# asd56585452/IGS

Measured on AMD Instinct MI355X. Metric: Gaussians rendered/sec (fwd+bwd) at 1352x1014; PSNR vs ref, higher is better.
Workload: dtype f32

## Files before the change

igs_amd/_cabi.py:

```python
import ctypes as C
import os

from . import build as _build

_LIB = None
E_RETRY = -6

ALLOC_FN = C.CFUNCTYPE(C.c_void_p, C.c_void_p, C.c_size_t)
_vp, _i, _f = C.c_void_p, C.c_int, C.c_float

class RefineStepArgs(C.Structure):
    _fields_ = [("stream", C.c_void_p),
                ("geometry_buffer", ALLOC_FN), ("geometry_user", C.c_void_p),
                ("binning_buffer", ALLOC_FN), ("binning_user", C.c_void_p),
                ("image_buffer", ALLOC_FN), ("image_user", C.c_void_p),
                ("workspace", C.c_void_p),
                ("P", C.c_int), ("D", C.c_int), ("M", C.c_int), ("width", C.c_int), ("height", C.c_int),
                ("background", C.c_void_p),
                ("param", C.c_void_p), ("exp_avg", C.c_void_p), ("exp_avg_sq", C.c_void_p), ("grad_out", C.c_void_p),
                ("off_xyz", C.c_size_t), ("off_rot", C.c_size_t), ("off_sh", C.c_size_t), ("off_opacity", C.c_size_t),
                ("off_scale", C.c_size_t),
                ("lr_xyz", C.c_float), ("lr_rot", C.c_float), ("lr_sh", C.c_float), ("lr_opacity", C.c_float), ("lr_scale", C.c_float),
                ("beta1", C.c_float), ("beta2", C.c_float), ("eps", C.c_float),
                ("step", C.c_int),
# ... 20 lines not shown

SIGNATURES = {
    "igs_rast_version": (_i, []),
    "igs_rast_last_error": (C.c_char_p, []),
    "igs_rast_forward": (_i, _FORWARD),
    "igs_rast_forward_async": (_i, _FORWARD),
    "igs_rast_forward_finish": (_i, []),
    "igs_rast_forward_nowait": (_i, _FORWARD),
    "igs_rast_last_status": (_i, _STATUS),
    "igs_rast_last_posted_status": (_i, _STATUS),
    "igs_rast_hint_scratch_clean": (None, [_i]),
    "igs_rast_count_gaussians": (_i, ([_vp, ALLOC_FN, _vp, ALLOC_FN, _vp, ALLOC_FN, _vp, _i, _i, _i, _vp, _i, _i]
                                      + [_vp] * 5 + [_f, _vp, _vp, _vp, _vp, _vp, _f, _f, _i] + [_vp] * 4 + [_i])),
    "igs_rast_set_slab_hint": (None, [_u]),
    "igs_rast_get_slab_hint": (_u, []),
    "igs_rast_backward_workspace_bytes": (_sz, [_i]),
    "igs_rast_backward": (_i, ([_vp, _i, _i, _i, _i, _vp, _i, _i] + [_vp] * 5 + [_f, _vp, _vp, _vp, _vp, _vp, _f, _f, _f]
                               + [_vp] * 5 + [_vp] * 7 + [_vp] + [_vp] * 8 + [_i, _i, _i])),
    "igs_rast_mark_visible": (_i, [_vp, _i, _vp, _vp, _vp, _vp]),
    "igs_rast_debug_dump": (_i, [_vp, _i, _i, _i, _i] + [_vp] * 8),
    "igs_rast_next_backward_options": (None, [_i, _f]),
    "igs_rast_nan_report_wait": (_i, []),
    "igs_rast_nan_report_handle": (_i, [_vp, _vp]),
    "igs_rast_nan_report_wait_at": (_i, [_vp, _u]),
    "igs_rast_last_backward_instance": (_i, []),
    "igs_rast_debug_poison_lds": (_i, [_vp]),
    "igs_rast_profile_enable": (_i, [_i]),
    "igs_rast_profile_read": (_i, [_vp, _vp, _vp, _vp, _i]),
    "igs_adam_step": (_i, [_vp, _sz, _vp, _vp, _vp, _vp, _f, _f, _f, _f, _f, _f]),
    "igs_adam_step_groups": (_i, [_vp, _i, _vp, _vp, _vp, _vp, _vp, _vp, _vp, _f, _f, _f, _f, _f]),
# ... 137 lines not shown
```

igs_amd/csrc/api.hip:

```cpp
#include <atomic>
#include "common.h"
#include "host_api.h"
#include <math.h>
#include <stdio.h>
#include <string.h>
#include <stdlib.h>
#include <time.h>

static thread_local char g_err[512] = "";
int fail(int code, const char* what, hipError_t e)
{
    if (e != hipSuccess) snprintf(g_err, sizeof g_err, "%s: %s", what, hipGetErrorString(e));
    else snprintf(g_err, sizeof g_err, "%s", what);
    return code;
}
int fail_in(const char* fn, const char* what)
{
    snprintf(g_err, sizeof g_err, "%s: %s", fn, what);
    return IGS_RAST_E_INVALID;
}
static const bool g_trace_launches = getenv("IGS_TRACE_LAUNCHES") != nullptr;
#define DBG_SYNC(what) do { if (debug || g_trace_launches) { hipError_t e_ = hipStreamSynchronize(s); if (e_ != hipSuccess) return fail(IGS_RAST_E_HIP, what, e_); \
                                                              if (g_trace_launches) { fprintf(stderr, "[igs] completed: %s\n", what); fflush(stderr); } } } while (0)

// ... 101 lines not shown
    if (r_sum) *r_sum = g_prof.r_sum;
    if (calls) *calls = g_prof.calls;
    if (reset) { for (int i = 0; i < ST_COUNT; i++) { g_prof.ms[i] = 0; g_prof.cnt[i] = 0; } g_prof.r_sum = 0; g_prof.calls = 0; }
    return ST_COUNT;
}

extern "C" int igs_rast_version(void) { return IGS_RAST_VERSION; }
extern "C" const char* igs_rast_last_error(void) { return g_err; }
static inline size_t ws_gacc_bytes(int P) { return ((size_t)(P > 0 ? P : 0) * GACC_F * 8 + 255) & ~(size_t)255; }
#define WS_LOSS_BYTES 4096
extern "C" size_t igs_rast_backward_workspace_bytes(int P) { return ws_gacc_bytes(P) + WS_LOSS_BYTES + 512; }

struct BinHint { uint32_t slab = 0; };
#define SLAB_MAX_BYTES (8ull << 30)
static thread_local BinHint g_hint;
static uint32_t slab_hint_for(uint32_t overflow)
{
    const uint64_t want = ((uint64_t)overflow + overflow / 4 + 255) / 256 * 256;
    return (uint32_t)(want > TILE_SORT_BIG ? TILE_SORT_BIG : want);
}
struct PendingFwd { bool active = false; uint32_t slab = 0; };
static thread_local PendingFwd g_pending;

struct FwdIn {
    hipStream_t s; igs_rast_alloc_fn geometry_buffer; void* geometry_user; igs_rast_alloc_fn binning_buffer; void* binning_user;
    igs_rast_alloc_fn image_buffer; void* image_user; int P, D, M; const float* background; int width, height;
    const float *means3D, *shs, *colors_precomp, *opacities, *scales; float scale_modifier; const float *rotations, *cov3D_precomp;
    const float *viewmatrix, *projmatrix, *cam_pos; float tan_fovx, tan_fovy, kernel_size; int prefiltered;
    float *out_color, *out_coord, *out_mcoord, *out_depth, *out_mdepth, *out_alpha, *out_normal; int* radii; int require_coord, require_depth, debug;
};
// ... 196 lines not shown
    if (b.pending) { g_host_seq = g_host_seq + 1 ? g_host_seq + 1 : 1; g_slot.pinned[3] = 0; }
    ba.host_seq = g_host_seq;
    if (b.pending && ex.no_latch) g_nowait_seq = g_host_seq;
    g_status_stream = s;
    if (ex.fused_ran) *ex.fused_ran = b.fuse_tiles;
    if (ex.count) {
        ba.tile_order = nullptr;
        HIP_TRY(launch_blend_count(s, ba, ex.count), "blend_count launch");
    } else if (b.fuse_tiles) {
        BlendBwdArgs& bb = *ex.fused_bwd;
        bb.W = in.width; bb.H = in.height; bb.gx = f.gx; bb.gy = f.gy; bb.fx = f.fp.fx; bb.fy = f.fp.fy; bb.bg = in.background;
        bb.ranges = b.ranges; bb.point_list = b.point_list; bb.rec = f.rec(); bb.colors_precomp = nullptr;
        bb.tile_order = nullptr;
        ba.tile_order = nullptr;
        if (b.step_order) { ba.step_order = f.ibuf(f.IL.tile_order); ba.reset_cursors = f.ibuf(f.IL.tile_count); }
        HIP_TRY(launch_blend_step(s, ba, bb, in.require_coord != 0, in.require_depth != 0, ex.fused_instance), "blend_step launch");
        if (b.step_order) g_counters_dirty = false;
    } else {
        HIP_TRY(launch_blend_fwd(s, ba, in.require_coord != 0, in.require_depth != 0), "blend_fwd launch");
    }
    DBG_SYNC("blend_fwd");
    prof_mark(s, ST_BLEND_FWD);
    return 0;
}

struct FrameStatus { uint32_t R, overflow, prefilter; };
static FrameStatus read_status(const uint32_t* p) { return { __atomic_load_n(&p[0], __ATOMIC_ACQUIRE), __atomic_load_n(&p[1], __ATOMIC_ACQUIRE), p[2] }; }
static int collect_status(hipStream_t s, uint32_t* overflow)
{
    if (int rc = wait_status(s)) return rc;
    const FrameStatus st = read_status(g_slot.pinned);
// ... 130 lines not shown
    const uint32_t seq = __atomic_load_n(&p[3], __ATOMIC_ACQUIRE);
    if (check_seq && seq != (g_nowait_seq ? g_nowait_seq : g_host_seq))
        return fail(IGS_RAST_E_RETRY, "igs_rast_last_status: the captured forward has not posted its status yet (replay the graph and synchronise the stream first)");
    const FrameStatus st = read_status(p);
    if (num_rendered) *num_rendered = st.R > 0x7FFFFFFFu ? 0x7FFFFFFF : (int)st.R;
    if (overflow) *overflow = st.overflow;
    if (prefilter_flag) *prefilter_flag = st.prefilter;
    if (st.overflow && slab_hint_for(st.overflow) > g_hint.slab) g_hint.slab = slab_hint_for(st.overflow);
    return 0;
}
extern "C" int igs_rast_last_status(int* num_rendered, unsigned* overflow, unsigned* prefilter) { return last_status(num_rendered, overflow, prefilter, true); }
extern "C" int igs_rast_last_posted_status(int* num_rendered, unsigned* overflow, unsigned* prefilter) { return last_status(num_rendered, overflow, prefilter, false); }

extern "C" void igs_rast_set_slab_hint(unsigned slots_per_tile) { g_hint.slab = slots_per_tile > TILE_SORT_BIG ? TILE_SORT_BIG : slots_per_tile; }
extern "C" unsigned igs_rast_get_slab_hint(void) { return g_hint.slab; }

static int g_last_bwd_instance = -1;
extern "C" int igs_rast_last_backward_instance(void) { return __atomic_load_n(&g_last_bwd_instance, __ATOMIC_RELAXED); }

#define NAN_RING 256
struct NanTicket { volatile uint32_t* word = nullptr; hipEvent_t ev = nullptr; uint32_t seq = 0; };
struct NanSlot { uint32_t* pinned = nullptr; uint32_t* pinned_dev = nullptr; NanTicket* tickets = nullptr; uint32_t seq = 0; bool requested = false; bool pending = false; };
static thread_local NanSlot g_nan[IGS_MAX_DEVICES];
static thread_local int g_nan_dev = -1;
static thread_local float g_next_clamp = 0.f;
extern "C" void igs_rast_next_backward_options(int nan_report, float clamp_grads)
{
    g_next_clamp = clamp_grads > 0.f ? clamp_grads : 0.f;
    int dev = 0;
    if (hipGetDevice(&dev) != hipSuccess || dev < 0 || dev >= IGS_MAX_DEVICES) return;
// ... 415 lines not shown
```

igs_amd/csrc/blend_bwd.hip:

```cpp
#include "blend_bwd_tile.h"

template <bool COORD, bool DEPTH, bool NORMAL, bool ABS = true, bool MASK = false>
__global__ void __launch_bounds__(256)
blend_bwd_kernel(const BlendBwdArgs a)
{
    using Cfg = BwdCfg<COORD, DEPTH, NORMAL, ABS>;
    __shared__ float4 chunk[Cfg::BCHUNK * Cfg::NQ];
    __shared__ uint32_t chunk_id[Cfg::BCHUNK];
    __shared__ uint64_t quad_bits[4][Cfg::NSW];
    __shared__ int wave_max[4];
    __shared__ __attribute__((aligned(16))) float red[Cfg::RED_FLOATS];

    uint32_t tile;
    if (a.tile_order && a.tile_order[a.gx * a.gy] == 1u) {
        if (blockIdx.x >= (uint32_t)(a.gx * a.gy)) return;
        tile = a.tile_order[blockIdx.x];
        if (tile >= (uint32_t)(a.gx * a.gy)) return;
    } else if (!tile_for_block(blockIdx.x, a.gx, a.gy, tile)) return;
    blend_bwd_tile<COORD, DEPTH, NORMAL, ABS, false, MASK>(a, tile, chunk, chunk_id, quad_bits, wave_max, red, nullptr);
}

hipError_t launch_blend_bwd(hipStream_t s, const BlendBwdArgs& a, bool coord, bool depth, bool* compact_layout, int* instance_bits)
{
    const dim3 grid(tile_grid_blocks(a.gx, a.gy)), block(256);
    const bool C = coord && (a.dL_dcoord || a.dL_dmcoord);
    const bool D = depth && (a.dL_ddepth || a.dL_dmdepth);
    const bool N = (coord || depth) && a.dL_dnormal;
    if (compact_layout) *compact_layout = !C && !D && !N;
    if (instance_bits) *instance_bits = (C ? 1 : 0) | (D ? 2 : 0) | (N ? 4 : 0) | ((C || (D && !N) || (!D && N) || a.want_absgrad) ? 8 : 0);
    if (a.first_trainable > 0) {
        if (C || a.want_absgrad || (D != N)) return hipErrorInvalidValue;
        if (D) hipLaunchKernelGGL((blend_bwd_kernel<false, true, true, false, true>), grid, block, 0, s, a);
        else   hipLaunchKernelGGL((blend_bwd_kernel<false, false, false, false, true>), grid, block, 0, s, a);
        return hipGetLastError();
// ... 14 lines not shown
```

igs_amd/csrc/blend_bwd_tile.h:

```cpp
#pragma once
#include "blend_common.h"
#include "blend_fwd_tile.h"

#define BCHUNK_MAX 128

template <int STRIDE_B, int R0, int N> struct ColWrite;
template <int STRIDE_B, int R0> struct ColWrite<STRIDE_B, R0, 1> {
    static __device__ __forceinline__ void run(unsigned m0, const float* v) {
        asm volatile("s_mov_b32 m0, %1\n\ts_nop 0\n\tds_write_addtid_b32 %0 offset:%2" :: "v"(v[R0]), "s"(m0), "n"(R0 * STRIDE_B) : "memory", "m0");
    }
};
template <int STRIDE_B, int R0> struct ColWrite<STRIDE_B, R0, 2> {
    static __device__ __forceinline__ void run(unsigned m0, const float* v) {
        asm volatile("s_mov_b32 m0, %2\n\ts_nop 0\n\tds_write_addtid_b32 %0 offset:%3\n\tds_write_addtid_b32 %1 offset:%4"
                     :: "v"(v[R0]), "v"(v[R0 + 1]), "s"(m0), "n"(R0 * STRIDE_B), "n"((R0 + 1) * STRIDE_B) : "memory", "m0");
    }
};
template <int STRIDE_B, int R0> struct ColWrite<STRIDE_B, R0, 3> {
    static __device__ __forceinline__ void run(unsigned m0, const float* v) {
        asm volatile("s_mov_b32 m0, %3\n\ts_nop 0\n\tds_write_addtid_b32 %0 offset:%4\n\tds_write_addtid_b32 %1 offset:%5\n\tds_write_addtid_b32 %2 offset:%6"
                     :: "v"(v[R0]), "v"(v[R0 + 1]), "v"(v[R0 + 2]), "s"(m0), "n"(R0 * STRIDE_B), "n"((R0 + 1) * STRIDE_B), "n"((R0 + 2) * STRIDE_B) : "memory", "m0");
    }
};
template <int STRIDE_B, int R0> struct ColWrite<STRIDE_B, R0, 4> {
// ... 34 lines not shown
        ColWrite<STRIDE_B, R0, 5>::run(m0, v);
        ColWrite<STRIDE_B, R0 + 5, N - 5>::run(m0, v);
    }
};

#define BWD_RED_STRIDE 68
template <bool COORD, bool DEPTH, bool NORMAL, bool ABS> struct BwdCfg {
    static constexpr bool GEO = COORD || DEPTH || NORMAL;
    static constexpr int NQ = GEO ? 6 : 3;
    static constexpr int BCHUNK = GEO ? 64 : 128;
    static constexpr int NSW = BCHUNK / 64;
    static constexpr int NROWS = 9 + (ABS ? 1 : 0) + (COORD ? 9 : 0) + (DEPTH ? 3 : 0) + (NORMAL ? 3 : 0);
    static constexpr int RED_FLOATS = 4 * NROWS * BWD_RED_STRIDE;
};

template <bool COORD, bool DEPTH, bool NORMAL, bool ABS, bool PRE, bool MASK = false>
__device__ __forceinline__ void blend_bwd_tile(const BlendBwdArgs& a, const uint32_t tile, float4* __restrict__ chunk, uint32_t* __restrict__ chunk_id,
                                               uint64_t (*quad_bits)[BwdCfg<COORD, DEPTH, NORMAL, ABS>::NSW], int* wave_max,
                                               float* __restrict__ red_all, const FwdPix* pre)
{
    constexpr bool GEO = COORD || DEPTH || NORMAL;
    constexpr int NQ = BwdCfg<COORD, DEPTH, NORMAL, ABS>::NQ;
    constexpr int BCHUNK = BwdCfg<COORD, DEPTH, NORMAL, ABS>::BCHUNK;
    constexpr int NSW = BwdCfg<COORD, DEPTH, NORMAL, ABS>::NSW;
    constexpr int NROWS = BwdCfg<COORD, DEPTH, NORMAL, ABS>::NROWS;
    constexpr int RED_STRIDE = BWD_RED_STRIDE;
    constexpr uint32_t SEG_ROT = NROWS == 9 ? 0x1b46bu
                               : NROWS == 10 ? 0x4431eu
                               : NROWS == 16 ? 0xa7dbb9c7u
                               : 0u;
    const uint32_t tx = tile % a.gx, ty = tile / a.gx;
    const uint32_t tid = threadIdx.x, lane = tid & 63, wid = tid >> 6;
    const uint32_t px = tx * TILE + (wid & 1) * 8 + (lane & 7);
    const uint32_t py = ty * TILE + (wid >> 1) * 8 + (lane >> 3);
    const bool inside = px < (uint32_t)a.W && py < (uint32_t)a.H;
    const float pixfx = (float)px, pixfy = (float)py;
    const float tile_x0 = (float)(tx * TILE), tile_y0 = (float)(ty * TILE);
    const size_t HW = (size_t)a.H * a.W;
    const size_t pix = (size_t)a.W * py + px;

    const uint2 range = ((const uint2*)a.ranges)[tile];
    int last_contributor;
    if constexpr (PRE) last_contributor = inside ? (int)min(pre->last_contributor, range.y - range.x) : 0;
    else last_contributor = inside ? (int)min(a.n_contrib[pix], range.y - range.x) : 0;
    uint32_t max_contributor = 0u;
    if constexpr (COORD || DEPTH) max_contributor = inside ? a.n_contrib[pix + HW] : 0u;

    float gp0 = 0, gp1 = 0, gp2 = 0, g_alpha = 0, T_final = 0, bg_dot = 0;
    if (a.l1_gt) {
        float acc = 0.f;
        if (inside) {
            float c0, c1, c2;
            if constexpr (PRE) {
                c0 = pre->C0 + pre->T * a.bg[0]; c1 = pre->C1 + pre->T * a.bg[1]; c2 = pre->C2 + pre->T * a.bg[2];
            } else { c0 = a.l1_color[pix]; c1 = a.l1_color[HW + pix]; c2 = a.l1_color[2 * HW + pix]; }
            const float d0 = c0 - a.l1_gt[pix], d1 = c1 - a.l1_gt[HW + pix];
// ... 44 lines not shown
                    gn0 = (d0 - dt * n0) / nlen; gn1 = (d1 - dt * n1) / nlen; gn2 = (d2 - dt * n2) / nlen;
                }
            }
        }
    }

    int my_wave_max;
    {
        int m = last_contributor;
#pragma unroll
        for (int off = 32; off > 0; off >>= 1) m = max(m, __shfl_xor(m, off, 64));
        if (lane == 0) wave_max[wid] = m;
        my_wave_max = __builtin_amdgcn_readfirstlane(m);
    }
    tile_barrier();
    const int n = max(max(wave_max[0], wave_max[1]), max(wave_max[2], wave_max[3]));
    const int rounds = (n + BCHUNK - 1) / BCHUNK;

    float T = T_final, S = 0.f, Dprev = 0.f, last_alpha = 0.f;
    const bool has_bg = (a.bg[0] != 0.f) || (a.bg[1] != 0.f) || (a.bg[2] != 0.f);
    const float halfW = 0.5f * a.W, halfH = 0.5f * a.H;
    float* myred = red_all + wid * (NROWS * RED_STRIDE);
    const unsigned myred_m0 = (unsigned)__builtin_amdgcn_readfirstlane((int)(unsigned)(size_t)myred);
    constexpr int LPR = NROWS <= 16 ? 4 : 2;
#ifndef BWD_ADJ
#define BWD_ADJ 1
#endif
    constexpr bool ADJ = BWD_ADJ && LPR == 4 && NROWS < 16;
    const int rrow = ADJ ? (int)(lane >> 2) : (int)(lane & (64 / LPR - 1)), rpart = ADJ ? (int)(lane & 3) : (int)(lane / (64 / LPR));
    const int rseg = ADJ ? rpart : LPR == 4 ? ((rpart + (int)((SEG_ROT >> (2 * (rrow & 15))) & 3u)) & 3) : rpart;
// ... 172 lines not shown
```

igs_amd/csrc/blend_fwd.hip:

```cpp
#include "blend_fwd_tile.h"

template <bool COORD, bool DEPTH, bool NORMAL, bool LEAN = false>
__global__ void __launch_bounds__(256) __attribute__((amdgpu_waves_per_eu(8, 8)))
blend_fwd_kernel(const BlendFwdArgs a)
{
    constexpr bool GEO = COORD || DEPTH || NORMAL;
    __shared__ float4 chunk[FWD_CHUNK * (GEO ? 6 : 3)];
    __shared__ uint64_t quad_bits[FWD_NLIST][FWD_NSW];
    __shared__ int wave_done[4];
    __shared__ uint32_t order_hist[2 * LOAD_CLASSES];

    if (blockIdx.x == 0 && threadIdx.x == 0 && a.host_dst) {
        __hip_atomic_store(&a.host_dst[0], a.stats_src[0], __ATOMIC_RELAXED, __HIP_MEMORY_SCOPE_SYSTEM);
        __hip_atomic_store(&a.host_dst[1], a.stats_src[1], __ATOMIC_RELAXED, __HIP_MEMORY_SCOPE_SYSTEM);
        __hip_atomic_store(&a.host_dst[2], a.flag_src[0], __ATOMIC_RELAXED, __HIP_MEMORY_SCOPE_SYSTEM);
        asm volatile("s_waitcnt vmcnt(0)" ::: "memory");
        __hip_atomic_store(&a.host_dst[3], a.host_seq, __ATOMIC_RELAXED, __HIP_MEMORY_SCOPE_SYSTEM);
    }
    if (blockIdx.x == 0 && a.tile_order) build_tile_order(a.ranges, (uint32_t)(a.gx * a.gy), a.tile_order, order_hist);
    uint32_t tile;
    if (!tile_for_block(blockIdx.x, a.gx, a.gy, tile)) return;
    FwdPix px;
    blend_fwd_tile<COORD, DEPTH, NORMAL, LEAN, true>(a, tile, chunk, quad_bits, wave_done, px);
}

hipError_t launch_blend_fwd(hipStream_t s, const BlendFwdArgs& a, bool coord, bool depth)
{
    const dim3 grid(tile_grid_blocks(a.gx, a.gy)), block(256);
    if (a.skip_bwd_state && coord && depth) hipLaunchKernelGGL((blend_fwd_kernel<true, true, true, true>), grid, block, 0, s, a);
    else if (coord && depth) hipLaunchKernelGGL((blend_fwd_kernel<true, true, true>), grid, block, 0, s, a);
    else if (coord) hipLaunchKernelGGL((blend_fwd_kernel<true, false, true>), grid, block, 0, s, a);
    else if (depth) hipLaunchKernelGGL((blend_fwd_kernel<false, true, true>), grid, block, 0, s, a);
    else hipLaunchKernelGGL((blend_fwd_kernel<false, false, false>), grid, block, 0, s, a);
    return hipGetLastError();
}
```

igs_amd/csrc/blend_fwd_tile.h:

```cpp
#pragma once
#include "blend_common.h"

#define FWD_CHUNK 192
#define FWD_NSW (FWD_CHUNK / 64)
#define FWD_NLIST 4

struct FwdPix {
    float C0, C1, C2;
    float T;
    float weight;
    uint32_t last_contributor;
};

template <bool COORD, bool DEPTH, bool NORMAL, bool LEAN, bool KEEP_N>
__device__ __forceinline__ void blend_fwd_tile(const BlendFwdArgs& a, const uint32_t tile, float4* __restrict__ chunk,
                                               uint64_t (*quad_bits)[FWD_NSW], int* wave_done, FwdPix& px_out)
{
    constexpr bool GEO = COORD || DEPTH || NORMAL;
    constexpr int NQ = GEO ? 6 : 3;
    const uint32_t tx = tile % a.gx, ty = tile / a.gx;
    const uint32_t tid = threadIdx.x, lane = tid & 63, wid = tid >> 6;
    const uint32_t px = tx * TILE + (wid & 1) * 8 + (lane & 7);
    const uint32_t py = ty * TILE + (wid >> 1) * 8 + (lane >> 3);
    const bool inside = px < (uint32_t)a.W && py < (uint32_t)a.H;
    const float pixfx = (float)px, pixfy = (float)py;
    const float tile_x0 = (float)(tx * TILE), tile_y0 = (float)(ty * TILE);

    const uint2 range = ((const uint2*)a.ranges)[tile];
    const int n = (int)(range.y - range.x);
    const int rounds = (n + FWD_CHUNK - 1) / FWD_CHUNK;

    float T = 1.0f;
    float Tl = inside ? 1.0f : 0.0f;
    uint32_t last_contributor = 0, max_contributor = 0xFFFFFFFFu;
    float C0 = 0, C1 = 0, C2 = 0, weight = 0;
    float Co0 = 0, Co1 = 0, Co2 = 0, mC0 = 0, mC1 = 0, mC2 = 0, Depth = 0, mDepth = 0, N0 = 0, N1 = 0, N2 = 0;

    if (tid < 4) wave_done[tid] = 0;
    for (int i = 0; i < rounds; i++) {
        tile_barrier();
        if (wave_done[0] & wave_done[1] & wave_done[2] & wave_done[3]) break;
        const int progress = i * FWD_CHUNK + (int)tid;
        uint32_t qmask = 0;
        if (tid < FWD_CHUNK && progress < n) {
            const uint32_t id = a.point_list[range.x + progress];
            const float4* src = (const float4*)(a.rec + (size_t)id * REC_F);
            float4 q0 = src[0], q1 = src[1], q2 = src[2];
            if (a.colors_precomp) {
                q1.z = a.colors_precomp[3 * (size_t)id]; q1.w = a.colors_precomp[3 * (size_t)id + 1];
                q2.x = a.colors_precomp[3 * (size_t)id + 2];
            }
            chunk[tid * NQ + 0] = q0; chunk[tid * NQ + 1] = q1; chunk[tid * NQ + 2] = q2;
// ... 3 lines not shown
        if (wid < FWD_NSW) {
#pragma unroll
            for (int q = 0; q < FWD_NLIST; q++) {
                const uint64_t b = __ballot((qmask >> q) & 1u);
                if (lane == 0) quad_bits[q][wid] = b;
            }
        }
        tile_barrier();
        auto blend_row = [&](const float4* r, const auto slot) {
                    const float4 q0 = r[0], q1 = r[1], q2 = r[2];
                    const float dx = q0.x - pixfx, dy = q0.y - pixfy;
                    const float power = gauss_power(q0.z, q0.w, q1.x, dx, dy);
                    const float alpha = fminf(0.99f, q1.y * __expf(power));
                    const float alpha_e = (!(power > 0.0f) && !(alpha < 1.0f / 255.0f)) ? alpha : 0.0f;
                    const float test_T = Tl * (1.0f - alpha_e);
                    const bool alive = !(test_T < 0.0001f);
                    const float aT = alive ? alpha_e * Tl : 0.0f;
                    const bool contrib = aT > 0.0f;
                    const uint32_t contributor = (uint32_t)(i * FWD_CHUNK + 1) + (uint32_t)slot;
                    C0 += q1.z * aT; C1 += q1.w * aT; C2 += q2.x * aT;
                    if constexpr (GEO) {
                        const float4 q3 = r[3];
                        const float4 q5 = r[5];
                        if constexpr (COORD) {
                            const float4 q4 = r[4];
                            const float c0 = q3.x + q4.x * dx + q4.y * dy;
                            const float c1 = q3.y + q4.z * dx + q4.w * dy;
                            const float c2 = q3.z + q5.x * dx + q5.y * dy;
                            Co0 += c0 * aT; Co1 += c1 * aT; Co2 += c2 * aT;
                        }
                        if constexpr (DEPTH) {
// ... 6 lines not shown
                    weight += aT;
                    T = alive ? test_T : T;
                    Tl = alive ? test_T : 0.0f;
                    last_contributor = contrib ? contributor : last_contributor;
        };
        if (__ballot(Tl != 0.0f) != 0ull) {
            bool wave_finished = false;
            for (int sw = 0; sw < FWD_NSW && !wave_finished; sw++) {
                uint64_t bits = uniform64(quad_bits[wid][sw]);
                while (bits != 0ull) {
                    const int jj = __builtin_ctzll(bits);
                    asm("s_bitset0_b64 %0, %1" : "+s"(bits) : "s"(jj));
                    const int j = sw * 64 + jj;
                    uint32_t addr;
                    if constexpr (NQ * 16 <= 64) asm("v_mul_u32_u24 %0, %1, %2" : "=v"(addr) : "s"(j), "n"(NQ * 16));
                    else asm("v_mul_u32_u24 %0, %1, %2" : "=v"(addr) : "s"(j), "v"(NQ * 16));
                    blend_row((const float4*)((const char*)chunk + addr), (uint32_t)j);
                }
                if (__ballot(Tl != 0.0f) == 0ull) wave_finished = true;
            }
        }
        const bool all_done = __ballot(Tl != 0.0f) == 0ull;
        if (lane == 0) wave_done[wid] = all_done ? 1 : 0;
    }

    if (inside) {
        const size_t HW = (size_t)a.H * a.W;
        const size_t pix = (size_t)a.W * py + px;
        if constexpr (GEO) {
            if (max_contributor != 0xFFFFFFFFu) {
                const uint32_t id = a.point_list[range.x + max_contributor - 1];
// ... 60 lines not shown
```

igs_amd/csrc/blend_step.hip:

```cpp
#include "blend_fwd_tile.h"
#include "blend_bwd_tile.h"

#ifdef BLEND_TIMELINE
#define BLEND_TL_MARKS 4
#define BLEND_TL_WGS 16384
__device__ unsigned long long g_blend_tl[BLEND_TL_WGS * BLEND_TL_MARKS];
extern "C" int igs_debug_blend_timeline(unsigned long long* host, int n)
{
    return (int)hipMemcpyFromSymbol(host, HIP_SYMBOL(g_blend_tl), (size_t)n * 8);
}
#define BTL(k, val) do { if (threadIdx.x == 0 && blockIdx.x < BLEND_TL_WGS) g_blend_tl[blockIdx.x * BLEND_TL_MARKS + (k)] = (val); } while (0)
#else
#define BTL(k, val) do { } while (0)
#endif
template <bool COORD, bool DEPTH, bool NORMAL, bool ABS, bool MASK = false>
__global__ void __launch_bounds__(256) __attribute__((amdgpu_waves_per_eu(8, 8)))
blend_step_kernel(const BlendFwdArgs f, const BlendBwdArgs b)
{
    constexpr bool GEO = COORD || DEPTH || NORMAL;
    using Cfg = BwdCfg<false, false, false, ABS>;
    constexpr size_t FWD_BYTES = (size_t)FWD_CHUNK * (GEO ? 6 : 3) * 16;
    constexpr size_t BWD_CHUNK_BYTES = (size_t)Cfg::BCHUNK * Cfg::NQ * 16;
    constexpr size_t BWD_BYTES = BWD_CHUNK_BYTES + (size_t)Cfg::RED_FLOATS * 4;
    __shared__ __attribute__((aligned(16))) char smem[FWD_BYTES > BWD_BYTES ? FWD_BYTES : BWD_BYTES];
    __shared__ uint64_t quad_bits_f[FWD_NLIST][FWD_NSW];
    __shared__ uint64_t quad_bits_b[4][Cfg::NSW];
    __shared__ int wave_done[4];
    __shared__ int wave_max[4];

    if (blockIdx.x == 0 && threadIdx.x == 0 && f.host_dst) {
        __hip_atomic_store(&f.host_dst[0], f.stats_src[0], __ATOMIC_RELAXED, __HIP_MEMORY_SCOPE_SYSTEM);
        __hip_atomic_store(&f.host_dst[1], f.stats_src[1], __ATOMIC_RELAXED, __HIP_MEMORY_SCOPE_SYSTEM);
        __hip_atomic_store(&f.host_dst[2], f.flag_src[0], __ATOMIC_RELAXED, __HIP_MEMORY_SCOPE_SYSTEM);
        asm volatile("s_waitcnt vmcnt(0)" ::: "memory");
        __hip_atomic_store(&f.host_dst[3], f.host_seq, __ATOMIC_RELAXED, __HIP_MEMORY_SCOPE_SYSTEM);
    }
    uint32_t tile;
    BTL(0, wall_clock64());
    if (f.step_order) {
        tile = f.step_order[blockIdx.x];
        if (tile >= (uint32_t)(f.gx * f.gy)) return;
    } else if (!tile_for_block(blockIdx.x, f.gx, f.gy, tile)) return;
    if (f.reset_cursors && threadIdx.x == 0) f.reset_cursors[tile] = 0u;
    BTL(3, (unsigned long long)(f.ranges[2 * tile + 1] - f.ranges[2 * tile]));
    FwdPix px;
    blend_fwd_tile<COORD, DEPTH, NORMAL, true, false>(f, tile, (float4*)smem, quad_bits_f, wave_done, px);
    tile_barrier();
    BTL(1, wall_clock64());
    blend_bwd_tile<false, false, false, ABS, true, MASK>(b, tile, (float4*)smem, nullptr, quad_bits_b, wave_max, (float*)(smem + BWD_CHUNK_BYTES), &px);
    BTL(2, wall_clock64());
}

hipError_t launch_blend_step(hipStream_t s, const BlendFwdArgs& f, const BlendBwdArgs& b, bool coord, bool depth, int* instance_bits)
{
    if (!f.skip_bwd_state || !b.l1_gt || b.dL_dcoord || b.dL_dmcoord || b.dL_ddepth || b.dL_dmdepth || b.dL_dnormal || b.dL_dalpha || b.colors_precomp)
        return hipErrorInvalidValue;
    const dim3 grid(tile_grid_blocks(f.gx, f.gy)), block(256);
    if (instance_bits) *instance_bits = b.want_absgrad ? 8 : 0;
    if (b.first_trainable > 0) {
        if (b.want_absgrad) return hipErrorInvalidValue;
        if (coord && depth) hipLaunchKernelGGL((blend_step_kernel<true, true, true, false, true>), grid, block, 0, s, f, b);
        else if (!coord && !depth) hipLaunchKernelGGL((blend_step_kernel<false, false, false, false, true>), grid, block, 0, s, f, b);
        else return hipErrorInvalidValue;
        return hipGetLastError();
    }
    if (coord && depth) {
        if (b.want_absgrad) hipLaunchKernelGGL((blend_step_kernel<true, true, true, true>), grid, block, 0, s, f, b);
        else hipLaunchKernelGGL((blend_step_kernel<true, true, true, false>), grid, block, 0, s, f, b);
    } else if (!coord && !depth) {
        if (b.want_absgrad) hipLaunchKernelGGL((blend_step_kernel<false, false, false, true>), grid, block, 0, s, f, b);
        else hipLaunchKernelGGL((blend_step_kernel<false, false, false, false>), grid, block, 0, s, f, b);
    } else return hipErrorInvalidValue;
    return hipGetLastError();
}
```

igs_amd/csrc/common.h:

```cpp
#pragma once
#include <hip/hip_runtime.h>
#include <stdint.h>
#include <stddef.h>

#define TILE 16
#define TILE_PIX 256
#define CHUNK 256

#define REC_F 32
#define REC_BLEND_F 24

#define GACC_F 32
#define GACC_COMPACT_F 16
enum { GA_COLOR = 0, GA_VP = 3, GA_CP = 6, GA_TS = 12, GA_RP = 13, GA_NRM = 15, GA_M2D = 18, GA_M2DZ = 20,
       GA_CONIC = 21, GA_OPA = 24, GA_USED = 25 };

static inline size_t align_up(size_t x, size_t a) { return (x + a - 1) / a * a; }

#define COUNTER_SHARDS 64
#define COUNTER_SHARD_STRIDE 16
#define SORT_ITEMS 8
#define SORT_TILE (256 * SORT_ITEMS)
#define SORT_MAX_PASSES 5
#define SORT_MAX_BLOCKS 256
// ... 109 lines not shown
hipError_t launch_count_score(hipStream_t s, int P, const int* count, const float* opacities, float* score);

struct BlendBwdArgs {
    int W, H, gx, gy;
    float fx, fy; const float* bg;
    const uint32_t* ranges; const uint32_t* point_list; const float* rec; const float* colors_precomp;
    const float *alphas, *normalmap, *accum_coord, *accum_depth, *normal_length; const uint32_t* n_contrib;
    const float *dL_dpix, *dL_dcoord, *dL_dmcoord, *dL_ddepth, *dL_dmdepth, *dL_dalpha, *dL_dnormal;
    double* gacc;
    const float *l1_color, *l1_gt; float l1_scale; float* l1_loss;
    int want_absgrad = 1;
    const uint32_t* tile_order = nullptr;
    int first_trainable = 0;
};
hipError_t launch_blend_bwd(hipStream_t s, const BlendBwdArgs& a, bool coord, bool depth, bool* compact_layout, int* instance_bits = nullptr);
hipError_t launch_blend_step(hipStream_t s, const BlendFwdArgs& f, const BlendBwdArgs& b, bool coord, bool depth, int* instance_bits = nullptr);

struct GeomBwdArgs {
    int P, D, M, W, H;
    const float *means3D, *shs, *scales, *rotations, *cov3D_precomp; const int* radii;
    float scale_modifier, tan_fovx, tan_fovy, fx, fy, kernel_size;
    const float *view, *proj, *campos;
    const float* rec; const double* gacc;
    int gacc_compact;
    float *dL_dmean2D, *dL_dcolor, *dL_dopacity, *dL_dmean3D, *dL_dcov3D, *dL_dsh, *dL_dscale, *dL_drot;
    uint32_t* nan_host = nullptr; uint32_t nan_seq = 0;
    float clamp = 0.f;
    const float* plane_cache = nullptr; uint32_t plane_tag = 0;
};
hipError_t launch_geom_bwd(hipStream_t s, const GeomBwdArgs& a);

// ... 183 lines not shown
```

include/igs_rast.h:

```cpp
#ifndef IGS_RAST_H
#define IGS_RAST_H

#include <stddef.h>
#include <stdint.h>

#ifdef __cplusplus
extern "C" {
#endif

#define IGS_RAST_VERSION 4

#define IGS_RAST_E_INVALID   (-1)
#define IGS_RAST_E_HIP       (-2)
#define IGS_RAST_E_ALLOC     (-3)
#define IGS_RAST_E_PREFILTER (-4)
#define IGS_RAST_E_CHANNELS  (-5)

#define IGS_RAST_E_RETRY     (-6)

typedef char* (*igs_rast_alloc_fn)(void* user, size_t bytes);

int igs_rast_version(void);
const char* igs_rast_last_error(void);

// ... 76 lines not shown
    const float* rotations,
    const float* cov3D_precomp,
    const float* viewmatrix,
    const float* projmatrix,
    const float* cam_pos,
    float tan_fovx, float tan_fovy,
    int prefiltered,
    float* out_color,
    int* count,
    float* score,
    int* radii,
    int debug);

void igs_rast_set_slab_hint(unsigned slots_per_tile);
unsigned igs_rast_get_slab_hint(void);

size_t igs_rast_backward_workspace_bytes(int P);

int igs_rast_backward(
    void* stream,
    int P, int D, int M, int R,
    const float* background,
    int width, int height,
    const float* means3D,
    const float* shs,
    const float* colors_precomp,
    const float* alphas,
    const float* scales,
    float scale_modifier,
    const float* rotations,
// ... 244 lines not shown
```

Before: 863.9 million.

## Turn fused blend step kernel into persistent tile loop with atomic ticket queues

The fused forward+backward blend kernel becomes persistent. The grid is sized to resident occupancy (CUs × blocks per CU), and workgroups pull tiles from eight sharded atomic ticket counters instead of launching one workgroup per tile. The next tile's range is prefetched with scalar loads after the backward barrier, and kernel arguments are reread from the kernarg segment through scalar loads to reduce register pressure. This aims to cut workgroup launch overhead and tail imbalance, but adds atomic contention and counter-reset logic that could fail at edge cases.

```diff
diff --git a/igs_amd/_cabi.py b/igs_amd/_cabi.py
--- a/igs_amd/_cabi.py
+++ b/igs_amd/_cabi.py
@@ -58,6 +58,7 @@
                                       + [_vp] * 5 + [_f, _vp, _vp, _vp, _vp, _vp, _f, _f, _i] + [_vp] * 4 + [_i])),
     "igs_rast_set_slab_hint": (None, [_u]),
     "igs_rast_get_slab_hint": (_u, []),
+    "igs_rast_set_step_grid": (_i, [_i]),
     "igs_rast_backward_workspace_bytes": (_sz, [_i]),
     "igs_rast_backward": (_i, ([_vp, _i, _i, _i, _i, _vp, _i, _i] + [_vp] * 5 + [_f, _vp, _vp, _vp, _vp, _vp, _f, _f, _f]
                                + [_vp] * 5 + [_vp] * 7 + [_vp] + [_vp] * 8 + [_i, _i, _i])),
diff --git a/igs_amd/csrc/api.hip b/igs_amd/csrc/api.hip
--- a/igs_amd/csrc/api.hip
+++ b/igs_amd/csrc/api.hip
@@ -139,6 +139,7 @@
 struct BinHint { uint32_t slab = 0; };
 #define SLAB_MAX_BYTES (8ull << 30)
 static thread_local BinHint g_hint;
+static std::atomic<int> g_step_grid{0};
 static uint32_t slab_hint_for(uint32_t overflow)
 {
     const uint64_t want = ((uint64_t)overflow + overflow / 4 + 255) / 256 * 256;
@@ -365,7 +366,8 @@
         bb.tile_order = nullptr;
         ba.tile_order = nullptr;
         if (b.step_order) { ba.step_order = f.ibuf(f.IL.tile_order); ba.reset_cursors = f.ibuf(f.IL.tile_count); }
-        HIP_TRY(launch_blend_step(s, ba, bb, in.require_coord != 0, in.require_depth != 0, ex.fused_instance), "blend_step launch");
+        HIP_TRY(launch_blend_step(s, ba, bb, in.require_coord != 0, in.require_depth != 0, ex.fused_instance, f.ibuf(f.IL.stats),
+                                  g_step_grid.load(std::memory_order_relaxed)), "blend_step launch");
         if (b.step_order) g_counters_dirty = false;
     } else {
         HIP_TRY(launch_blend_fwd(s, ba, in.require_coord != 0, in.require_depth != 0), "blend_fwd launch");
@@ -526,6 +528,12 @@
 
 extern "C" void igs_rast_set_slab_hint(unsigned slots_per_tile) { g_hint.slab = slots_per_tile > TILE_SORT_BIG ? TILE_SORT_BIG : slots_per_tile; }
 extern "C" unsigned igs_rast_get_slab_hint(void) { return g_hint.slab; }
+extern "C" int igs_rast_set_step_grid(int n)
+{
+    if (n < -1) return fail(IGS_RAST_E_INVALID, "igs_rast_set_step_grid: n must be -1 (no tile loop), 0 (automatic) or a workgroup count");
+    g_step_grid.store(n, std::memory_order_relaxed);
+    return 0;
+}
 
 static int g_last_bwd_instance = -1;
 extern "C" int igs_rast_last_backward_instance(void) { return __atomic_load_n(&g_last_bwd_instance, __ATOMIC_RELAXED); }
diff --git a/igs_amd/csrc/blend_bwd.hip b/igs_amd/csrc/blend_bwd.hip
--- a/igs_amd/csrc/blend_bwd.hip
+++ b/igs_amd/csrc/blend_bwd.hip
@@ -17,7 +17,7 @@
         tile = a.tile_order[blockIdx.x];
         if (tile >= (uint32_t)(a.gx * a.gy)) return;
     } else if (!tile_for_block(blockIdx.x, a.gx, a.gy, tile)) return;
-    blend_bwd_tile<COORD, DEPTH, NORMAL, ABS, false, MASK>(a, tile, chunk, chunk_id, quad_bits, wave_max, red, nullptr);
+    blend_bwd_tile<COORD, DEPTH, NORMAL, ABS, false, MASK>(a, tile, ((const uint2*)a.ranges)[tile], threadIdx.x, chunk, chunk_id, quad_bits, wave_max, red, nullptr);
 }
 
 hipError_t launch_blend_bwd(hipStream_t s, const BlendBwdArgs& a, bool coord, bool depth, bool* compact_layout, int* instance_bits)
diff --git a/igs_amd/csrc/blend_bwd_tile.h b/igs_amd/csrc/blend_bwd_tile.h
--- a/igs_amd/csrc/blend_bwd_tile.h
+++ b/igs_amd/csrc/blend_bwd_tile.h
@@ -72,10 +72,11 @@
     static constexpr int RED_FLOATS = 4 * NROWS * BWD_RED_STRIDE;
 };
 
-template <bool COORD, bool DEPTH, bool NORMAL, bool ABS, bool PRE, bool MASK = false>
-__device__ __forceinline__ void blend_bwd_tile(const BlendBwdArgs& a, const uint32_t tile, float4* __restrict__ chunk, uint32_t* __restrict__ chunk_id,
-                                               uint64_t (*quad_bits)[BwdCfg<COORD, DEPTH, NORMAL, ABS>::NSW], int* wave_max,
-                                               float* __restrict__ red_all, const FwdPix* pre)
+struct BwdNoHook { __device__ __forceinline__ void operator()() const {} };
+template <bool COORD, bool DEPTH, bool NORMAL, bool ABS, bool PRE, bool MASK = false, class Hook = BwdNoHook>
+__device__ __forceinline__ void blend_bwd_tile(const BlendBwdArgs& a, const uint32_t tile, const uint2 range, const uint32_t tid, float4* __restrict__ chunk,
+                                               uint32_t* __restrict__ chunk_id, uint64_t (*quad_bits)[BwdCfg<COORD, DEPTH, NORMAL, ABS>::NSW],
+                                               int* wave_max, float* __restrict__ red_all, const FwdPix* pre, Hook after_barrier = Hook())
 {
     constexpr bool GEO = COORD || DEPTH || NORMAL;
     constexpr int NQ = BwdCfg<COORD, DEPTH, NORMAL, ABS>::NQ;
@@ -88,7 +89,7 @@
                                : NROWS == 16 ? 0xa7dbb9c7u
                                : 0u;
     const uint32_t tx = tile % a.gx, ty = tile / a.gx;
-    const uint32_t tid = threadIdx.x, lane = tid & 63, wid = tid >> 6;
+    const uint32_t lane = tid & 63, wid = tid >> 6;
     const uint32_t px = tx * TILE + (wid & 1) * 8 + (lane & 7);
     const uint32_t py = ty * TILE + (wid >> 1) * 8 + (lane >> 3);
     const bool inside = px < (uint32_t)a.W && py < (uint32_t)a.H;
@@ -97,7 +98,6 @@
     const size_t HW = (size_t)a.H * a.W;
     const size_t pix = (size_t)a.W * py + px;
 
-    const uint2 range = ((const uint2*)a.ranges)[tile];
     int last_contributor;
     if constexpr (PRE) last_contributor = inside ? (int)min(pre->last_contributor, range.y - range.x) : 0;
     else last_contributor = inside ? (int)min(a.n_contrib[pix], range.y - range.x) : 0;
@@ -172,6 +172,7 @@
         my_wave_max = __builtin_amdgcn_readfirstlane(m);
     }
     tile_barrier();
+    after_barrier();
     const int n = max(max(wave_max[0], wave_max[1]), max(wave_max[2], wave_max[3]));
     const int rounds = (n + BCHUNK - 1) / BCHUNK;
 
diff --git a/igs_amd/csrc/blend_fwd.hip b/igs_amd/csrc/blend_fwd.hip
--- a/igs_amd/csrc/blend_fwd.hip
+++ b/igs_amd/csrc/blend_fwd.hip
@@ -21,7 +21,7 @@
     uint32_t tile;
     if (!tile_for_block(blockIdx.x, a.gx, a.gy, tile)) return;
     FwdPix px;
-    blend_fwd_tile<COORD, DEPTH, NORMAL, LEAN, true>(a, tile, chunk, quad_bits, wave_done, px);
+    blend_fwd_tile<COORD, DEPTH, NORMAL, LEAN, true>(a, tile, ((const uint2*)a.ranges)[tile], threadIdx.x, chunk, quad_bits, wave_done, px);
 }
 
 hipError_t launch_blend_fwd(hipStream_t s, const BlendFwdArgs& a, bool coord, bool depth)
diff --git a/igs_amd/csrc/blend_fwd_tile.h b/igs_amd/csrc/blend_fwd_tile.h
--- a/igs_amd/csrc/blend_fwd_tile.h
+++ b/igs_amd/csrc/blend_fwd_tile.h
@@ -13,20 +13,19 @@
 };
 
 template <bool COORD, bool DEPTH, bool NORMAL, bool LEAN, bool KEEP_N>
-__device__ __forceinline__ void blend_fwd_tile(const BlendFwdArgs& a, const uint32_t tile, float4* __restrict__ chunk,
+__device__ __forceinline__ void blend_fwd_tile(const BlendFwdArgs& a, const uint32_t tile, const uint2 range, const uint32_t tid, float4* __restrict__ chunk,
                                                uint64_t (*quad_bits)[FWD_NSW], int* wave_done, FwdPix& px_out)
 {
     constexpr bool GEO = COORD || DEPTH || NORMAL;
     constexpr int NQ = GEO ? 6 : 3;
     const uint32_t tx = tile % a.gx, ty = tile / a.gx;
-    const uint32_t tid = threadIdx.x, lane = tid & 63, wid = tid >> 6;
+    const uint32_t lane = tid & 63, wid = tid >> 6;
     const uint32_t px = tx * TILE + (wid & 1) * 8 + (lane & 7);
     const uint32_t py = ty * TILE + (wid >> 1) * 8 + (lane >> 3);
     const bool inside = px < (uint32_t)a.W && py < (uint32_t)a.H;
     const float pixfx = (float)px, pixfy = (float)py;
     const float tile_x0 = (float)(tx * TILE), tile_y0 = (float)(ty * TILE);
 
-    const uint2 range = ((const uint2*)a.ranges)[tile];
     const int n = (int)(range.y - range.x);
     const int rounds = (n + FWD_CHUNK - 1) / FWD_CHUNK;
 
@@ -36,6 +35,10 @@
     float C0 = 0, C1 = 0, C2 = 0, weight = 0;
     float Co0 = 0, Co1 = 0, Co2 = 0, mC0 = 0, mC1 = 0, mC2 = 0, Depth = 0, mDepth = 0, N0 = 0, N1 = 0, N2 = 0;
 
+    float alive_min;
+    asm volatile("s_mov_b32 %0, 0x38d1b717" : "=s"(alive_min));
+    uint32_t rec_stride = 0;
+    if constexpr (NQ * 16 > 64) asm volatile("v_mov_b32 %0, %1" : "=v"(rec_stride) : "n"(NQ * 16));
     if (tid < 4) wave_done[tid] = 0;
     for (int i = 0; i < rounds; i++) {
         tile_barrier();
@@ -69,7 +72,7 @@
                     const float alpha = fminf(0.99f, q1.y * __expf(power));
                     const float alpha_e = (!(power > 0.0f) && !(alpha < 1.0f / 255.0f)) ? alpha : 0.0f;
                     const float test_T = Tl * (1.0f - alpha_e);
-                    const bool alive = !(test_T < 0.0001f);
+                    const bool alive = !(test_T < alive_min);
                     const float aT = alive ? alpha_e * Tl : 0.0f;
                     const bool contrib = aT > 0.0f;
                     const uint32_t contributor = (uint32_t)(i * FWD_CHUNK + 1) + (uint32_t)slot;
@@ -106,7 +109,7 @@
                     const int j = sw * 64 + jj;
                     uint32_t addr;
                     if constexpr (NQ * 16 <= 64) asm("v_mul_u32_u24 %0, %1, %2" : "=v"(addr) : "s"(j), "n"(NQ * 16));
-                    else asm("v_mul_u32_u24 %0, %1, %2" : "=v"(addr) : "s"(j), "v"(NQ * 16));
+                    else asm("v_mul_u32_u24 %0, %1, %2" : "=v"(addr) : "s"(j), "v"(rec_stride));
                     blend_row((const float4*)((const char*)chunk + addr), (uint32_t)j);
                 }
                 if (__ballot(Tl != 0.0f) == 0ull) wave_finished = true;
diff --git a/igs_amd/csrc/blend_step.hip b/igs_amd/csrc/blend_step.hip
--- a/igs_amd/csrc/blend_step.hip
+++ b/igs_amd/csrc/blend_step.hip
@@ -1,5 +1,7 @@
 #include "blend_fwd_tile.h"
 #include "blend_bwd_tile.h"
+#include <atomic>
+#include <cstdlib>
 
 #ifdef BLEND_TIMELINE
 #define BLEND_TL_MARKS 4
@@ -9,13 +11,37 @@
 {
     return (int)hipMemcpyFromSymbol(host, HIP_SYMBOL(g_blend_tl), (size_t)n * 8);
 }
-#define BTL(k, val) do { if (threadIdx.x == 0 && blockIdx.x < BLEND_TL_WGS) g_blend_tl[blockIdx.x * BLEND_TL_MARKS + (k)] = (val); } while (0)
+#define BTL(k, val) do { if (threadIdx.x == 0 && ticket < BLEND_TL_WGS) g_blend_tl[ticket * BLEND_TL_MARKS + (k)] = (val); } while (0)
 #else
 #define BTL(k, val) do { } while (0)
 #endif
+
+struct StepLoop { uint32_t* ticket; uint32_t total, queues; };
+#define STEP_TICKET_WORD 16
+
+typedef const __attribute__((address_space(4))) uint32_t* step_cptr;
+__device__ __forceinline__ uint32_t step_sload(const uint32_t* p, uint32_t i) { return ((step_cptr)(uintptr_t)p)[i]; }
+
+typedef const __attribute__((address_space(4))) char* step_kptr;
+constexpr size_t STEP_KARG_BWD = (sizeof(BlendFwdArgs) + alignof(BlendBwdArgs) - 1) / alignof(BlendBwdArgs) * alignof(BlendBwdArgs);
+template <class T> __device__ __forceinline__ T step_karg(size_t offset)
+{
+    step_kptr k = (step_kptr)__builtin_amdgcn_kernarg_segment_ptr();
+    uint32_t lo = (uint32_t)(uintptr_t)k, hi = (uint32_t)((uintptr_t)k >> 32);
+    asm volatile("" : "+s"(lo), "+s"(hi));
+    k = (step_kptr)(((uintptr_t)(uint32_t)__builtin_amdgcn_readfirstlane((int)hi) << 32) | (uint32_t)__builtin_amdgcn_readfirstlane((int)lo));
+    static_assert(sizeof(T) % 4 == 0, "kernel arguments are read word by word");
+    uint32_t w[sizeof(T) / 4];
+#pragma unroll
+    for (size_t i = 0; i < sizeof(T) / 4; i++) w[i] = ((step_cptr)(k + offset))[i];
+    T v;
+    __builtin_memcpy(&v, w, sizeof(T));
+    return v;
+}
+
 template <bool COORD, bool DEPTH, bool NORMAL, bool ABS, bool MASK = false>
 __global__ void __launch_bounds__(256) __attribute__((amdgpu_waves_per_eu(8, 8)))
-blend_step_kernel(const BlendFwdArgs f, const BlendBwdArgs b)
+blend_step_kernel(const BlendFwdArgs f, const BlendBwdArgs b_unused, const StepLoop lp)
 {
     constexpr bool GEO = COORD || DEPTH || NORMAL;
     using Cfg = BwdCfg<false, false, false, ABS>;
@@ -27,6 +53,7 @@
     __shared__ uint64_t quad_bits_b[4][Cfg::NSW];
     __shared__ int wave_done[4];
     __shared__ int wave_max[4];
+    __shared__ uint32_t next_slot;
 
     if (blockIdx.x == 0 && threadIdx.x == 0 && f.host_dst) {
         __hip_atomic_store(&f.host_dst[0], f.stats_src[0], __ATOMIC_RELAXED, __HIP_MEMORY_SCOPE_SYSTEM);
@@ -35,41 +62,105 @@
         asm volatile("s_waitcnt vmcnt(0)" ::: "memory");
         __hip_atomic_store(&f.host_dst[3], f.host_seq, __ATOMIC_RELAXED, __HIP_MEMORY_SCOPE_SYSTEM);
     }
-    uint32_t tile;
-    BTL(0, wall_clock64());
-    if (f.step_order) {
-        tile = f.step_order[blockIdx.x];
-        if (tile >= (uint32_t)(f.gx * f.gy)) return;
-    } else if (!tile_for_block(blockIdx.x, f.gx, f.gy, tile)) return;
-    if (f.reset_cursors && threadIdx.x == 0) f.reset_cursors[tile] = 0u;
-    BTL(3, (unsigned long long)(f.ranges[2 * tile + 1] - f.ranges[2 * tile]));
-    FwdPix px;
-    blend_fwd_tile<COORD, DEPTH, NORMAL, true, false>(f, tile, (float4*)smem, quad_bits_f, wave_done, px);
-    tile_barrier();
-    BTL(1, wall_clock64());
-    blend_bwd_tile<false, false, false, ABS, true, MASK>(b, tile, (float4*)smem, nullptr, quad_bits_b, wave_max, (float*)(smem + BWD_CHUNK_BYTES), &px);
-    BTL(2, wall_clock64());
+    const uint32_t ntiles = (uint32_t)(f.gx * f.gy);
+    auto tile_of_slot = [&](const uint32_t slot) -> uint32_t {
+        if (slot >= lp.total) return 0xFFFFFFFFu;
+        if (f.step_order) return step_sload(f.step_order, slot);
+        uint32_t t;
+        return tile_for_block(slot, (uint32_t)f.gx, (uint32_t)f.gy, t) ? t : 0xFFFFFFFFu;
+    };
+    auto range_of_tile = [&](const uint32_t t) -> uint2 {
+        if (t >= ntiles) return make_uint2(0u, 0u);
+        return make_uint2(step_sload(f.ranges, 2u * t), step_sload(f.ranges, 2u * t + 1u));
+    };
+    const uint32_t queue = blockIdx.x & (lp.queues - 1u);
+    const uint32_t queue_wgs = (gridDim.x - queue + lp.queues - 1u) / lp.queues;
+    uint32_t ticket = blockIdx.x;
+    if (ticket >= lp.total) return;
+    uint32_t tile = tile_of_slot(ticket);
+    uint2 range = range_of_tile(tile);
+    for (;;) {
+        const bool work = tile < ntiles;
+        BTL(0, wall_clock64());
+        uint32_t drawn = 0u;
+        if (lp.ticket && threadIdx.x == 0) drawn = __hip_atomic_fetch_add(&lp.ticket[queue], 1u, __ATOMIC_RELAXED, __HIP_MEMORY_SCOPE_AGENT);
+        uint32_t tid = threadIdx.x;
+        asm volatile("" : "+v"(tid));
+        FwdPix px;
+        if (work) {
+            const BlendFwdArgs f = step_karg<BlendFwdArgs>(0);
+            if (f.reset_cursors && threadIdx.x == 0) f.reset_cursors[tile] = 0u;
+            BTL(3, (unsigned long long)(range.y - range.x));
+            blend_fwd_tile<COORD, DEPTH, NORMAL, true, false>(f, tile, range, tid, (float4*)smem, quad_bits_f, wave_done, px);
+        }
+        if (lp.ticket && threadIdx.x == 0) {
+            if (drawn == lp.total / lp.queues - 1u) __hip_atomic_store(&lp.ticket[queue], 0u, __ATOMIC_RELAXED, __HIP_MEMORY_SCOPE_AGENT);
+            next_slot = (queue_wgs + drawn) * lp.queues + queue;
+        }
+        tile_barrier();
+        BTL(1, wall_clock64());
+        const uint32_t slot_n = lp.ticket ? (uint32_t)__builtin_amdgcn_readfirstlane((int)next_slot) : lp.total;
+        const uint32_t tile_n = tile_of_slot(slot_n);
+        uint2 range_n;
+        if (work) {
+            blend_bwd_tile<false, false, false, ABS, true, MASK>(step_karg<BlendBwdArgs>(STEP_KARG_BWD), tile, range, tid, (float4*)smem, nullptr, quad_bits_b, wave_max,
+                                                                 (float*)(smem + BWD_CHUNK_BYTES), &px,
+                                                                 [&]() { range_n = range_of_tile(tile_n); });
+        } else range_n = range_of_tile(tile_n);
+        BTL(2, wall_clock64());
+        if (slot_n >= lp.total) return;
+        ticket = slot_n; tile = tile_n; range = range_n;
+        tile_barrier();
+    }
 }
 
-hipError_t launch_blend_step(hipStream_t s, const BlendFwdArgs& f, const BlendBwdArgs& b, bool coord, bool depth, int* instance_bits)
+template <bool COORD, bool DEPTH, bool NORMAL, bool ABS, bool MASK>
+static hipError_t launch_step_instance(hipStream_t s, const BlendFwdArgs& f, const BlendBwdArgs& b, uint32_t* stats, int step_grid)
+{
+    const auto kernel = blend_step_kernel<COORD, DEPTH, NORMAL, ABS, MASK>;
+    static std::atomic<int> resident_wgs[16];
+    static const bool one_queue = getenv("IGS_STEP_ONE_QUEUE") != nullptr;
+    const uint32_t total = tile_grid_blocks(f.gx, f.gy);
+    StepLoop lp{ nullptr, total, 1u };
+    uint32_t grid = total;
+    if (step_grid >= 0 && stats) {
+        if (step_grid > 0) grid = (uint32_t)step_grid;
+        else {
+            int dev = 0;
+            if (hipError_t e = hipGetDevice(&dev)) return e;
+            int cached = (unsigned)dev < 16u ? resident_wgs[dev].load(std::memory_order_relaxed) : 0;
+            if (!cached) {
+                int per_cu = 0, cus = 0;
+                if (hipError_t e = hipOccupancyMaxActiveBlocksPerMultiprocessor(&per_cu, kernel, 256, 0)) return e;
+                if (hipError_t e = hipDeviceGetAttribute(&cus, hipDeviceAttributeMultiprocessorCount, dev)) return e;
+                cached = per_cu > 0 && cus > 0 ? per_cu * cus : 1;
+                if ((unsigned)dev < 16u) resident_wgs[dev].store(cached, std::memory_order_relaxed);
+            }
+            grid = (uint32_t)cached;
+        }
+        if (step_grid > 0 || grid < total) { lp.ticket = stats + STEP_TICKET_WORD; lp.queues = (one_queue || grid < 8u) ? 1u : 8u; }
+        else grid = total;
+    }
+    hipLaunchKernelGGL(kernel, dim3(grid), dim3(256), 0, s, f, b, lp);
+    return hipGetLastError();
+}
+
+hipError_t launch_blend_step(hipStream_t s, const BlendFwdArgs& f, const BlendBwdArgs& b, bool coord, bool depth, int* instance_bits,
+                             uint32_t* stats, int step_grid)
 {
     if (!f.skip_bwd_state || !b.l1_gt || b.dL_dcoord || b.dL_dmcoord || b.dL_ddepth || b.dL_dmdepth || b.dL_dnormal || b.dL_dalpha || b.colors_precomp)
         return hipErrorInvalidValue;
-    const dim3 grid(tile_grid_blocks(f.gx, f.gy)), block(256);
     if (instance_bits) *instance_bits = b.want_absgrad ? 8 : 0;
+    if (coord != depth) return hipErrorInvalidValue;
     if (b.first_trainable > 0) {
         if (b.want_absgrad) return hipErrorInvalidValue;
-        if (coord && depth) hipLaunchKernelGGL((blend_step_kernel<true, true, true, false, true>), grid, block, 0, s, f, b);
-        else if (!coord && !depth) hipLaunchKernelGGL((blend_step_kernel<false, false, false, false, true>), grid, block, 0, s, f, b);
-        else return hipErrorInvalidValue;
-        return hipGetLastError();
+        if (coord) return launch_step_instance<true, true, true, false, true>(s, f, b, stats, step_grid);
+        return launch_step_instance<false, false, false, false, true>(s, f, b, stats, step_grid);
     }
-    if (coord && depth) {
-        if (b.want_absgrad) hipLaunchKernelGGL((blend_step_kernel<true, true, true, true>), grid, block, 0, s, f, b);
-        else hipLaunchKernelGGL((blend_step_kernel<true, true, true, false>), grid, block, 0, s, f, b);
-    } else if (!coord && !depth) {
-        if (b.want_absgrad) hipLaunchKernelGGL((blend_step_kernel<false, false, false, true>), grid, block, 0, s, f, b);
-        else hipLaunchKernelGGL((blend_step_kernel<false, false, false, false>), grid, block, 0, s, f, b);
-    } else return hipErrorInvalidValue;
-    return hipGetLastError();
+    if (coord) {
+        if (b.want_absgrad) return launch_step_instance<true, true, true, true, false>(s, f, b, stats, step_grid);
+        return launch_step_instance<true, true, true, false, false>(s, f, b, stats, step_grid);
+    }
+    if (b.want_absgrad) return launch_step_instance<false, false, false, true, false>(s, f, b, stats, step_grid);
+    return launch_step_instance<false, false, false, false, false>(s, f, b, stats, step_grid);
 }
diff --git a/igs_amd/csrc/common.h b/igs_amd/csrc/common.h
--- a/igs_amd/csrc/common.h
+++ b/igs_amd/csrc/common.h
@@ -147,7 +147,8 @@
     int first_trainable = 0;
 };
 hipError_t launch_blend_bwd(hipStream_t s, const BlendBwdArgs& a, bool coord, bool depth, bool* compact_layout, int* instance_bits = nullptr);
-hipError_t launch_blend_step(hipStream_t s, const BlendFwdArgs& f, const BlendBwdArgs& b, bool coord, bool depth, int* instance_bits = nullptr);
+hipError_t launch_blend_step(hipStream_t s, const BlendFwdArgs& f, const BlendBwdArgs& b, bool coord, bool depth, int* instance_bits = nullptr,
+                             uint32_t* stats = nullptr, int step_grid = 0);
 
 struct GeomBwdArgs {
     int P, D, M, W, H;
diff --git a/include/igs_rast.h b/include/igs_rast.h
--- a/include/igs_rast.h
+++ b/include/igs_rast.h
@@ -114,6 +114,8 @@
 
 void igs_rast_set_slab_hint(unsigned slots_per_tile);
 unsigned igs_rast_get_slab_hint(void);
+
+int igs_rast_set_step_grid(int n);
 
 size_t igs_rast_backward_workspace_bytes(int P);
 
```

Result: slower. 730.1 million (-15.5%).
